# tirtho109/parallel_AMG

Measured on AMD Instinct MI355X. Metric: V-cycle iters/sec + fine-SpMV HBM GB/s, 3D Poisson 128M dofs at 1/2/4/8 GPU, higher is better.
Workload: dtype f64; 1 GPU; poisson3d 512^3 fp64, SA-AMG V(1,1) weighted-Jacobi, 1 part(s); n=134217728, nnz_fine=937951232, levels=6, max_coarse=1000, parallelism=row-slab partition p1

## Files before the change

include/pamg.h:

```cpp
#ifndef PAMG_H
#define PAMG_H

#include <stdint.h>

#ifdef __cplusplus
extern "C" {
#endif

#define PAMG_OK 0
#define PAMG_E_ARG (-1)
#define PAMG_E_HIP (-2)
#define PAMG_E_RCCL (-3)
#define PAMG_E_OVERFLOW (-4)
#define PAMG_E_SETUP (-5)
#define PAMG_E_STATE (-6)
#define PAMG_E_NOMEM (-7)

typedef struct pamg_ctx pamg_ctx;
typedef struct pamg_plan pamg_plan;
typedef struct pamg_vec pamg_vec;
typedef struct pamg_mat pamg_mat;
typedef struct pamg_hier pamg_hier;
typedef struct pamg_hcsr pamg_hcsr;

// ... 55 lines not shown
int pamg_mat_upload(pamg_ctx* ctx, int64_t nrows, int64_t ncols_local, const int64_t* rowptr,
                    const void* col, int col_is_64, const double* val, int index_base,
                    const pamg_plan* col_plan, pamg_mat** out);
int pamg_mat_upload_perm(pamg_ctx* ctx, int64_t nrows, int64_t ncols_local, const int64_t* rowptr,
                         const void* col, int col_is_64, const double* val, int index_base,
                         const pamg_plan* col_plan, const int64_t* row_perm,
                         const int64_t* col_perm, pamg_mat** out);
int pamg_mat_upload_blocked(pamg_ctx* ctx, int64_t nrows, int64_t ncols_local, const int64_t* rowptr,
                            const void* col, int col_is_64, const double* val, int index_base,
                            const pamg_plan* col_plan, int bs, pamg_mat** out);
int pamg_mat_destroy(pamg_mat* A);
int pamg_mat_info(const pamg_mat* A, int64_t* nrows, int64_t* ncols_local, int64_t* nnz);
int pamg_mat_stream_bytes(const pamg_mat* A, int64_t* bytes);
int pamg_mat_layout(const pamg_mat* A, int set, int out[10]);
int pamg_mat_ell_window(const pamg_mat* A, int out[16]);
int pamg_mat_ell_classes(const pamg_mat* A, int64_t out[8]);

int pamg_mat_set_block_diag(pamg_ctx* ctx, pamg_mat* A, int bs, const double* blocks, const double* inv);
int pamg_mat_block_size(const pamg_mat* A, int* bs);

int pamg_spmv(pamg_ctx* ctx, const pamg_mat* A, pamg_vec* x, pamg_vec* y);
int pamg_residual(pamg_ctx* ctx, const pamg_mat* A, pamg_vec* x, const pamg_vec* b,
                  pamg_vec* r, double* nrm2);
int pamg_jacobi(pamg_ctx* ctx, const pamg_mat* A, pamg_vec* x, const pamg_vec* b,
                pamg_vec* tmp, double omega, int nsweeps);
int pamg_jacobi_residual(pamg_ctx* ctx, const pamg_mat* A, pamg_vec* x, const pamg_vec* b,
                         pamg_vec* t, pamg_vec* r, double omega, int* fused);
int pamg_chebyshev_coeffs(double lmax, double ratio, int degree, double* c1, double* c2);
int pamg_chebyshev(pamg_ctx* ctx, const pamg_mat* A, pamg_vec* x, const pamg_vec* b, pamg_vec* tmp1,
                   pamg_vec* tmp2, double lmax, double ratio, int degree);
// ... 86 lines not shown
```

parallel_amg_amd/_lib.py:

```python
from __future__ import annotations

import contextlib
import ctypes as C
import os

_HERE = os.path.dirname(os.path.abspath(__file__))
LIB_PATH = os.environ.get("PAMG_LIB") or os.path.join(_HERE, "libpamg.so")

PAMG_OK = 0
ERRORS = {-1: "PAMG_E_ARG", -2: "PAMG_E_HIP", -3: "PAMG_E_RCCL", -4: "PAMG_E_OVERFLOW",
          -5: "PAMG_E_SETUP", -6: "PAMG_E_STATE", -7: "PAMG_E_NOMEM"}


class PamgError(RuntimeError):
    def __init__(self, code, fn, msg):
        super().__init__(f"{fn} -> {ERRORS.get(code, code)}: {msg}")
        self.code = code


vp = C.c_void_p
i32, i64, dbl = C.c_int, C.c_int64, C.c_double
pvp = C.POINTER(C.c_void_p)
pi64 = C.POINTER(C.c_int64)
pdbl = C.POINTER(C.c_double)
# ... 39 lines not shown
    "pamg_vec_copy": [vp, vp, vp],
    "pamg_vec_axpby": [vp, dbl, vp, dbl, vp],
    "pamg_vec_dot": [vp, vp, vp, pdbl],
    "pamg_vec_nrm2": [vp, vp, pdbl],
    "pamg_exchange": [vp, vp, vp],
    "pamg_exchange_begin": [vp, vp, vp],
    "pamg_exchange_end": [vp, vp, vp],
    "pamg_mat_upload": [vp, i64, i64, vp, vp, i32, vp, i32, vp, pvp],
    "pamg_mat_upload_perm": [vp, i64, i64, vp, vp, i32, vp, i32, vp, vp, vp, pvp],
    "pamg_mat_upload_blocked": [vp, i64, i64, vp, vp, i32, vp, i32, vp, i32, pvp],
    "pamg_mat_destroy": [vp],
    "pamg_mat_info": [vp, pi64, pi64, pi64],
    "pamg_mat_stream_bytes": [vp, pi64],
    "pamg_mat_layout": [vp, i32, C.POINTER(C.c_int)],
    "pamg_mat_ell_window": [vp, C.POINTER(C.c_int)],
    "pamg_mat_ell_classes": [vp, pi64],
    "pamg_mat_set_block_diag": [vp, vp, i32, vp, vp],
    "pamg_mat_block_size": [vp, C.POINTER(C.c_int)],
    "pamg_spmv": [vp, vp, vp, vp],
    "pamg_residual": [vp, vp, vp, vp, vp, pdbl],
    "pamg_jacobi": [vp, vp, vp, vp, vp, dbl, i32],
    "pamg_jacobi_residual": [vp, vp, vp, vp, vp, vp, dbl, pi32],
    "pamg_chebyshev_coeffs": [dbl, dbl, i32, vp, vp],
    "pamg_chebyshev": [vp, vp, vp, vp, vp, vp, dbl, dbl, i32],
    "pamg_estimate_lmax": [vp, vp, vp, vp, i32, i32, vp],
    "pamg_block_jacobi": [vp, vp, vp, vp, vp, dbl, i32],
    "pamg_block_chebyshev": [vp, vp, vp, vp, vp, vp, dbl, dbl, i32],
    "pamg_estimate_lmax_block": [vp, vp, vp, vp, i32, i32, vp],
    "pamg_hier_set_omega": [vp, vp],
    "pamg_hier_create": [vp, i32, vp, vp, vp, vp, i64, vp, i32, vp, pvp],
# ... 94 lines not shown
    old = C.c_int64()
    call("pamg_get_option", key.encode(), C.byref(old))
    call("pamg_set_option", key.encode(), int(value))
    try:
        yield
    finally:
        call("pamg_set_option", key.encode(), old.value)


def layout_of(M, part_set: int = 0) -> dict:
    out = (C.c_int * 10)()
    call("pamg_mat_layout", M.handle, part_set, out)
    win = (C.c_int * 16)()
    if part_set == 0:
        call("pamg_mat_ell_window", M.handle, win)
    cls = (C.c_int64 * 8)()
    if part_set == 0:
        call("pamg_mat_ell_classes", M.handle, cls)
    return {"ell_class": bool(cls[0]),
            "ell_class_census": {"slices": int(cls[1]), "classes_mean": round(cls[2] / max(cls[1], 1), 2),
                                 "classes_max": int(cls[3]), "record_bytes": int(cls[4]), "id_bytes": int(cls[5]),
                                 "replaced_bytes": int(cls[6])},
            "ell_xwin": bool(win[0]), "ell_xwin_groups": int(win[1]), "ell_gather_groups": int(win[2]),
            "ell_xwin_max_window": int(win[3]), "ell_xwin_noncontig_groups": int(win[4]),
            "ell_xwin_max_pairs": int(win[5]), "ell_xwin_max_chunks": int(win[6]),
            "ell_xwin_census": {"groups": int(win[7]), "full_groups": int(win[13]), "window_mean": int(win[8]),
                                "window_p95": int(win[9]), "runs_mean": int(win[10]), "runs_max": int(win[11]),
                                "pairs_mean": int(win[12])},
            "c24": bool(out[0]), "vd": bool(out[1]), "rl8": bool(out[2]), "cd": int(out[3]),
            "cd_offsets": int(out[4]), "tm": bool(out[5]), "tm_rs": int(out[6]),
            "tile_nnz": int(out[7]), "tiles": int(out[8]), "anchored": bool(out[9] & 1), "per_tile": bool(out[9] & 2),
            "x_stage": bool(out[9] & 4), "sym": bool(out[9] & 8), "sym_rows": 2 if out[9] & 16 else 1,
            "jr_fused": bool(out[9] & 32), "tm_vd": bool(out[9] & 64), "sym_vd": bool(out[9] & 128),
            "ell": bool(out[9] & 512), "pnc": bool(out[9] & 1024),
            "rpat": bool(out[9] & 2048), "pnc_compact": bool(out[9] & 4096),
            "ell_pair": bool(out[9] & 8192), "pnc_tiled": bool(out[9] & 16384),
            "bsr": bool(out[9] & 32768)}


def last_error() -> str:
    return lib().pamg_last_error().decode(errors="replace")


# ... 3 lines not shown
```

parallel_amg_amd/csrc/kernels.hip:

```cpp

#include "pamg_device.h"
#include "div_rn.h"

namespace pamg {
namespace {

__device__ __forceinline__ int wave_incl_scan(int v) {
    const int lane = threadIdx.x & 63, rl = lane & 15;
    int t;
    t = __builtin_amdgcn_mov_dpp(v, 0x111, 0xf, 0xf, false);
    if (rl >= 1) v += t;
    t = __builtin_amdgcn_mov_dpp(v, 0x112, 0xf, 0xf, false);
    if (rl >= 2) v += t;
    t = __builtin_amdgcn_mov_dpp(v, 0x114, 0xf, 0xf, false);
    if (rl >= 4) v += t;
    t = __builtin_amdgcn_mov_dpp(v, 0x118, 0xf, 0xf, false);
    if (rl >= 8) v += t;
    t = __builtin_amdgcn_mov_dpp(v, 0x142, 0xf, 0xf, false);
    if (lane & 16) v += t;
    t = __builtin_amdgcn_mov_dpp(v, 0x143, 0xf, 0xf, false);
    if (lane >= 32) v += t;
    return v;
}

// ... 1553 lines not shown
    for (int e = 0; e < 4; ++e) {
        const bool ok = FULL || 4 * q + e < L;
        const double p = vv[e] * xv[e];
        const double t = s + p;
        s = ok ? t : s;
    }
}

constexpr int kEllwPre = 12;
__device__ __forceinline__ void ellw_load(uint32_t (&cq)[kEllwPre], const uint32_t* __restrict__ cw, int first, int nq,
                                          int q0, int stride) {
#pragma unroll
    for (int e = 0; e < kEllwPre; ++e) cq[e] = cw[nq > 0 ? first + min(q0 + e, nq - 1) * stride : 0];
}

template <int OP, bool CLS>
__global__ __launch_bounds__(kEllGroup) void k_rows_ellw(int nrows, const int4* __restrict__ gslices,
                                                         const int2* __restrict__ smeta, const uint32_t* __restrict__ cw,
                                                         const uint8_t* __restrict__ cid,
                                                         const uint8_t* __restrict__ len, const uint8_t* __restrict__ dpos,
                                                         const int4* __restrict__ gmeta, const int* __restrict__ otab,
                                                         const double* __restrict__ vtab, const int4* __restrict__ wmeta, const int2* __restrict__ chunks,
                                                         const uint16_t* __restrict__ lofs, int win, int gather_all,
                                                         int ngroups, const double* __restrict__ x,
                                                         const double* __restrict__ b, double* __restrict__ y,
                                                         double omega, double c1 = 0.0,
                                                         const double* __restrict__ xold = nullptr) {
    extern __shared__ double ellw_lds[];
    double* lx = ellw_lds;
    double* lv = ellw_lds + win;
    uint16_t* lof = reinterpret_cast<uint16_t*>(lv + 256);
    const int per = (ngroups + 7) / 8;
    const int g = (blockIdx.x & 7) * per + (blockIdx.x >> 3);
    if (g >= ngroups) return;
    const int tid = threadIdx.x, lane = tid & 63;
    const int w = __builtin_amdgcn_readfirstlane(tid >> 6);
    const int4 gm = gmeta[g], wm = wmeta[g], gs = gslices[g];
    const int np = gm.y;
    const bool windowed = wm.y > 0 && !gather_all;
    const double vtv = vtab[gm.x + (tid < np ? tid : 0)];
    const uint32_t* __restrict__ l32 = reinterpret_cast<const uint32_t*>(lofs + wm.z);
    const uint32_t la = l32[windowed && tid < 2 * np ? tid : 0], lb = l32[windowed && tid + 256 < 2 * np ? tid + 256 : 0];
    const int2 cmv = chunks[wm.x + (w + 4 * lane < wm.y ? w + 4 * lane : 0)];
    const int slice = w == 0 ? gs.x : w == 1 ? gs.y : w == 2 ? gs.z : gs.w;
    const int i = slice * kEllW + lane;
    const bool in = slice >= 0 && i < nrows;
    const int ic = in ? i : 0;
    const int L = in ? (int)len[ic] : 0;
    const int2 sm = smeta[slice >= 0 ? slice : 0];
    const int nq = slice >= 0 ? ((CLS ? sm.y & 0xff : sm.y) + 3) >> 2 : 0;
    const int nfull = CLS && slice >= 0 ? __builtin_amdgcn_readfirstlane(((sm.y >> 8) & 0xff) >> 2) : 0;
    const int stride = CLS ? sm.y >> 16 : kEllW;
    const int first = sm.x + (CLS ? (in ? (int)cid[ic] : 0) : lane);
    const uint32_t* __restrict__ cp = cw + first;
    double pb = 0.0, px = 0.0, py = 0.0, pxo = 0.0;
    if constexpr (OP == OP_RESID || kDiagOp<OP>) pb = b[ic];
    if constexpr (kDiagOp<OP>) px = x[ic];
    if constexpr (OP == OP_PROLONG) py = y[ic];
    if constexpr (OP == OP_CHEB) pxo = xold ? xold[ic] : 0.0;
    uint32_t dkw = 0u;
    int dk = 255;
    if constexpr (kDiagOp<OP>) {
        dk = in ? (int)dpos[ic] : 255;
        dkw = cw[dk != 255 ? first + (dk >> 2) * stride : 0];
    }
    double s = 0.0;
    if (windowed) {
        uint32_t cq[kEllwPre];
        ellw_load(cq, cw, first, nq, 0, stride);
        for (int k = 0; w + 4 * k < wm.y; ++k) {
            const int col = __builtin_amdgcn_readlane(cmv.x, k), sc = __builtin_amdgcn_readlane(cmv.y, k);
            if (lane < (sc >> 16))
                __builtin_amdgcn_global_load_lds(
                    (const __attribute__((address_space(1))) void*)(x + col + 2 * lane),
                    (__attribute__((address_space(3))) void*)(lx + (sc & 0xffff)), 16, 0, 0);
        }
        if (tid < np) lv[tid] = vtv;
        if (tid < 2 * np) reinterpret_cast<uint32_t*>(lof)[tid] = la;
        if (tid + 256 < 2 * np) reinterpret_cast<uint32_t*>(lof)[tid + 256] = lb;
        __syncthreads();
        for (int q0 = 0; q0 < nq; q0 += kEllwPre) {
            if (q0 > 0) ellw_load(cq, cw, first, nq, q0, stride);
#pragma unroll
            for (int e = 0; e < kEllwPre; ++e)
                if (CLS && q0 + e < nfull)
// ... 959 lines not shown
template <int OP>
void launch_rows_op(const pamg_mat& A, const TileSet& ts, const double* x, const double* b,
                    double* y, double omega, hipStream_t s, Cheb ch = Cheb{}) {
    if (ts.bsr) launch_bsr<OP, 0>(A, x, b, y, omega, s, ch);
    if (ts.sym) launch_sym<OP>(A, x, b, y, omega, s, ch);
    if (ts.ell) {
        const EllSet& E = A.ell;
        const int grid = (int)((E.ngroups + 7) / 8 * 8);
        auto go = [&](auto kern) {
            kern<<<grid, kEllGroup, 0, s>>>((int)A.nrows, E.d_gorder, E.d_anc, E.d_smeta, E.d_ci, E.d_vi, E.d_len,
                                            E.d_gmeta, E.d_otab, E.d_vtab, (int)E.ngroups, x, b, y, omega, ch.c1,
                                            ch.xold);
        };
        if (E.win) {
            const int win = std::max(E.max_window, 128);
            const size_t lds = sizeof(double) * (size_t)(win + 256) + sizeof(uint16_t) * 4 * 256;
            auto gow = [&](auto kern) {
                kern<<<grid, kEllGroup, lds, s>>>((int)A.nrows, E.d_gslices, E.d_smeta, E.d_ci, E.d_cid, E.d_len, E.d_dpos,
                                                  E.d_gmeta, E.d_otab, E.d_vtab, E.d_wmeta, E.d_chunks, E.d_lof, win,
                                                  (reinterpret_cast<uintptr_t>(x) & 15) != 0 ? 1 : 0, (int)E.ngroups, x, b,
                                                  y, omega, ch.c1, ch.xold);
            };
            if (E.cls) gow(k_rows_ellw<OP, true>);
            else gow(k_rows_ellw<OP, false>);
        } else if (E.d_anc) {
            if (E.paired) go(k_rows_ell<OP, true, true>);
            else go(k_rows_ell<OP, true, false>);
        } else {
            if (E.paired) go(k_rows_ell<OP, false, true>);
            else go(k_rows_ell<OP, false, false>);
        }
    }
    if constexpr (OP != OP_CHEB) {
        if (ts.pnc) launch_pnc<OP>(A, x, b, y, omega, s);
        if (ts.rpat) launch_rpat<OP>(A, x, b, y, omega, s);
    }
    if (ts.n_short > 0) {
        if (ts.tile_nnz == 1024) launch_tile<OP, 1024>(A, ts, x, b, y, omega, s, ch);
        else if (ts.tile_nnz == 4096) launch_tile<OP, 4096>(A, ts, x, b, y, omega, s, ch);
// ... 379 lines not shown
```

parallel_amg_amd/csrc/matrix.hip:

```cpp
#include <algorithm>
#include <array>
#include <atomic>
#include <chrono>
#include <cstdint>
#include <cstdio>
#include <cstdlib>
#include <cstring>
#include <functional>
#include <iterator>
#include <memory>
#include <mutex>
#include <new>
#include <thread>
#include <utility>
#include <vector>

#include "pamg_device.h"
#include "pamg_host.h"

namespace {

int host_threads() {
    static const int n = [] {
        const char* e = std::getenv("OMP_NUM_THREADS");
        int v = e ? std::atoi(e) : 0;
        if (v <= 0) v = (int)std::thread::hardware_concurrency();
        return std::max(1, std::min(v, 64));
    }();
    return n;
}

template <class F>
void par_for(int64_t n, F&& f) {
// ... 784 lines not shown
                couple(take);
            }
            for (int t : touched) score[t] = 0;
            grp.push_back(g);
        }
    }
    std::vector<std::vector<std::pair<int, int>>>().swap(scoup);
    std::vector<std::vector<uint64_t>>().swap(spair);
    const int64_t ng = (int64_t)grp.size();
    std::vector<std::vector<int>> goff(ng);
    std::vector<std::vector<uint64_t>> gval(ng);
    std::vector<std::vector<int2>> gchunk(ng);
    std::vector<std::vector<uint16_t>> glof(ng);
    std::vector<int> gwin(ng, 0), gruns(ng, 0);
    std::vector<int64_t> gnnz(ng, 0);
    std::vector<uint32_t> cw(words + 1, 0u);
    std::vector<uint8_t> len(n + kVecPad, 0), dpos(n + kVecPad, (uint8_t)255);
    par_for(ng, [&](int64_t a, int64_t b) {
        constexpr int kSlots = 1024;
        std::vector<int> pid(kSlots), pstamp(kSlots, -1), pkey_o(kSlots);
        std::vector<uint64_t> pkey_v(kSlots);
        std::vector<int> o, lmin(4 * 256), lmax(4 * 256);
        std::vector<uint64_t> v;
        std::vector<std::array<int, 2>> rng;
        std::vector<std::array<int, 3>> runs;
        for (int64_t g = a; g < b && ok; ++g) {
            const int stamp = (int)(g - a);
            o.clear();
            v.clear();
            for (int w = 0; w < 4 && ok; ++w) {
// ... 56 lines not shown
            }
            int slots = 0, nch = 0;
            for (auto& r : runs) {
                r[2] = slots;
                slots += r[1] - r[0];
                nch += (r[1] - r[0] + 127) / 128;
            }
            if (slots == 0 || slots > cap || nch > pamg::kEllWinChunks) continue;
            if (runs.front()[0] < 0 || runs.back()[1] > ((int)A->ncols + 1)) continue;
            gwin[g] = slots;
            gruns[g] = (int)runs.size();
            for (const auto& r : runs)
                for (int c = r[0]; c < r[1]; c += 128)
                    gchunk[g].push_back(make_int2(c, (r[2] + c - r[0]) | (std::min(128, r[1] - c) / 2) << 16));
            glof[g].assign((size_t)4 * np, (uint16_t)64);
            for (int w = 0; w < 4; ++w)
                for (int p = 0; p < np; ++p) {
                    uint16_t word = 64;
                    if (grp[g][w] >= 0 && lmax[w * 256 + p] >= 0) {
                        const int c0 = grp[g][w] * kEllW + o[p], c = c0 + lmin[w * 256 + p];
                        size_t r = 0;
                        while (r + 1 < runs.size() && runs[r + 1][0] <= c) ++r;
                        word = (uint16_t)(runs[r][2] + c0 - runs[r][0] + 64);
                    }
                    glof[g][(size_t)w * np + p] = word;
                }
        }
    });
    if (!ok) return PAMG_OK;
    {
        int64_t have = 0;
        for (int64_t g = 0; g < ng; ++g) have += gwin[g] > 0;
        for (int k = 8; k >= 2 && have > 0; --k) {
            const int fit = ((pamg::kEllLdsPerCu / k - 2048) / 8 - 256) & ~1;
            int64_t keep = 0;
            for (int64_t g = 0; g < ng; ++g) keep += gwin[g] > 0 && gwin[g] <= fit;
            if (keep * 100 < pamg::kEllWinKeep * have) continue;
            for (int64_t g = 0; g < ng; ++g)
                if (gwin[g] > fit) {
                    gwin[g] = 0;
                    gchunk[g].clear();
                    glof[g].clear();
                }
            break;
        }
    }
    pamg::EllSet& E = A->ell;
    int64_t win_nnz = 0, win_slots = 0, win_runs = 0, win_pairs = 0;
    for (int64_t g = 0; g < ng; ++g) {
        E.max_pairs = std::max(E.max_pairs, (int)goff[g].size());
        bool contig = true;
        for (int w = 1; w < 4; ++w) contig = contig && (grp[g][w] < 0 || grp[g][w] == grp[g][0] + w);
        if (gwin[g] > 0) {
            ++E.win_groups;
            win_nnz += gnnz[g];
            win_slots += gwin[g];
            E.max_window = std::max(E.max_window, gwin[g]);
// ... 9 lines not shown
    }
    if ((int64_t)E.win_groups * 100 < pamg::kEllWinMinShare * ng || win_nnz * 100 < pamg::kEllWinMinRatio100 * win_slots) {
        E = pamg::EllSet{};
        return PAMG_OK;
    }
    {
        std::vector<int> ws;
        for (int64_t g = 0; g < ng; ++g)
            if (gwin[g] > 0) ws.push_back(gwin[g]);
        std::sort(ws.begin(), ws.end());
        E.p95_window = ws[(ws.size() - 1) * 95 / 100];
        E.mean_window = (int)(win_slots / E.win_groups);
        E.mean_runs = (int)(win_runs / E.win_groups);
        E.mean_pairs = (int)(win_pairs / E.win_groups);
    }
    std::vector<int4> gmeta(ng), wmeta(ng), gsl(ng);
    int64_t on = 0, cn = 0, ln = 0;
    for (int64_t g = 0; g < ng; ++g) {
        const int np = (int)goff[g].size();
        gmeta[g] = make_int4((int)on, np, (int)on, np);
        wmeta[g] = make_int4((int)cn, (int)gchunk[g].size(), (int)ln, gwin[g]);
        gsl[g] = make_int4(grp[g][0], grp[g][1], grp[g][2], grp[g][3]);
        on += np;
        cn += (int64_t)gchunk[g].size();
        ln += (int64_t)glof[g].size();
    }
    if (ln >= INT32_MAX || cn >= INT32_MAX) {
        E = pamg::EllSet{};
        return PAMG_OK;
    }
    std::vector<int> otab(on + 1, 0);
    std::vector<double> vtab(on + 1, 0.0);
    std::vector<int2> chunks(cn + 1, make_int2(0, 0));
    std::vector<uint16_t> lof(ln + 2, (uint16_t)0);
    par_for(ng, [&](int64_t a, int64_t b) {
        for (int64_t g = a; g < b; ++g) {
            std::copy(goff[g].begin(), goff[g].end(), otab.begin() + gmeta[g].x);
            for (size_t e = 0; e < gval[g].size(); ++e) std::memcpy(&vtab[gmeta[g].x + e], &gval[g][e], 8);
            std::copy(gchunk[g].begin(), gchunk[g].end(), chunks.begin() + wmeta[g].x);
            std::copy(glof[g].begin(), glof[g].end(), lof.begin() + wmeta[g].z);
        }
    });
    std::vector<int2> smeta_c;
    std::vector<uint32_t> ccw;
    std::vector<uint8_t> cid;
    if (pamg::options().ell_xwin == 1) {
        std::vector<int> snc(ns, 0), smin(ns, 0);
        cid.assign(n + kVecPad, 0);
        par_for(ns, [&](int64_t a, int64_t b) {
            int rep[kEllW];
            for (int64_t q = a; q < b; ++q) {
                const int nq = (smeta[q].y + 3) / 4;
                const int64_t r0 = q * kEllW, s0 = smeta[q].x;
                const int rows = (int)std::min<int64_t>(n - r0, kEllW);
                int nc = 0;
                for (int l = 0; l < rows; ++l) {
                    int c = 0;
                    for (; c < nc; ++c) {
                        const int m = rep[c];
                        bool same = len[r0 + l] == len[r0 + m] && dpos[r0 + l] == dpos[r0 + m];
                        for (int k = 0; k < nq && same; ++k) same = cw[s0 + (int64_t)k * kEllW + l] == cw[s0 + (int64_t)k * kEllW + m];
// ... 63 lines not shown
    CHECK(dalloc(&E.d_wmeta, ng));
    CHECK(dalloc(&E.d_chunks, cn + 1));
    CHECK(dalloc(&E.d_lof, ln + 2));
    CHECK(dalloc(&E.d_dpos, n + kVecPad));
    CHECK(h2d(ctx, E.d_dpos, dpos.data(), dpos.size()));
    CHECK(h2d(ctx, E.d_smeta, sm_up.data(), sizeof(int2) * ns));
    CHECK(h2d(ctx, E.d_ci, cw_up.data(), sizeof(uint32_t) * (up_words + 1)));
    CHECK(h2d(ctx, E.d_len, len.data(), len.size()));
    CHECK(h2d(ctx, E.d_gmeta, gmeta.data(), sizeof(int4) * ng));
    CHECK(h2d(ctx, E.d_otab, otab.data(), sizeof(int) * (on + 1)));
    CHECK(h2d(ctx, E.d_vtab, vtab.data(), sizeof(double) * (on + 1)));
    CHECK(h2d(ctx, E.d_gslices, gsl.data(), sizeof(int4) * ng));
    CHECK(h2d(ctx, E.d_wmeta, wmeta.data(), sizeof(int4) * ng));
    CHECK(h2d(ctx, E.d_chunks, chunks.data(), sizeof(int2) * (cn + 1)));
    CHECK(h2d(ctx, E.d_lof, lof.data(), sizeof(uint16_t) * (ln + 2)));
    A->interior.ell = true;
    return PAMG_OK;
}

int build_ell(pamg_mat* A, const PtrVec& rp, const IdxVec& ci, const double* val,
              bool anchored, const std::vector<int>& inner) {
    using pamg::kEllGroup;
    using pamg::kEllSkip;
    using pamg::kEllW;
    const int64_t n = A->nrows;
    std::vector<char> in_set;
    if ((int64_t)inner.size() != n) {
        in_set.assign(n, 0);
        for (int i : inner) in_set[i] = 1;
    }
// ... 194 lines not shown
        (int64_t)u.inner.size() * 4 >= (int64_t)nrows * 3 && nrows >= pamg::options().ell_min_rows &&
        (n_own_cols == nrows || pamg::options().ell_restrict)) {
        CHECK(build_ell(A, u.rp, u.ci, u.val, n_own_cols != nrows, u.inner));
        if (A->interior.ell) u.inner.clear();
        u.tr.mark("ell");
    }
    return PAMG_OK;
}

int64_t ell_bytes(const pamg_mat* A) {
    if (!A->interior.ell) return 0;
    const int64_t nrows = A->nrows;
    const int64_t index = A->ell.cls ? 4 * A->ell.cls_words + nrows : (A->ell.paired ? 4 : 8) * A->ell.words;
    return index + nrows + 8 * A->ell.nslices + 16 * A->ell.ngroups + 4 * A->ell.otab_n +
           8 * A->ell.vtab_n + (A->ell.d_anc ? 4 * nrows : 0) +
           (A->ell.win ? 32 * A->ell.ngroups + 8 * A->ell.nchunks + 2 * A->ell.lof_n + nrows : 0);
}

void ell_report(const pamg_mat* A, const pamg::TileSet& t, int out[10]) {
    if (!t.ell) return;
    out[8] = (int)A->ell.ngroups;
    out[9] |= 512 | (A->ell.paired ? 8192 : 0);
}

void ell_window(const pamg_mat* A, int out[16]) {
    const pamg::EllSet& E = A->ell;
    const bool w = A->interior.ell && E.win;
    out[0] = w ? 1 : 0;
    out[1] = w ? E.win_groups : 0;
    out[2] = w ? E.gather_groups : 0;
    out[3] = w ? E.max_window : 0;
    out[4] = w ? E.noncontig_groups : 0;
    out[5] = w ? E.max_pairs : 0;
    out[6] = w ? E.max_chunks : 0;
    out[7] = w ? (int)E.ngroups : 0;
    out[8] = w ? E.mean_window : 0;
    out[9] = w ? E.p95_window : 0;
    out[10] = w ? E.mean_runs : 0;
    out[11] = w ? E.max_runs : 0;
    out[12] = w ? E.mean_pairs : 0;
    out[13] = w ? E.full_groups : 0;
    out[14] = out[15] = 0;
}

void ell_classes(const pamg_mat* A, int64_t out[8]) {
    const pamg::EllSet& E = A->ell;
    const bool c = A->interior.ell && E.cls;
    out[0] = c ? 1 : 0;
    out[1] = c ? E.nslices : 0;
    out[2] = c ? E.cls_total : 0;
    out[3] = c ? E.cls_max : 0;
    out[4] = c ? 4 * E.cls_words : 0;
    out[5] = c ? A->nrows : 0;
    out[6] = c ? 4 * E.words : 0;
    out[7] = 0;
}

void ell_free(pamg::EllSet& E) {
    dfree(E.d_cid);
    dfree(E.d_gorder);
    dfree(E.d_smeta);
    dfree(E.d_ci);
    dfree(E.d_vi);
    dfree(E.d_len);
    dfree(E.d_gmeta);
    dfree(E.d_otab);
    dfree(E.d_vtab);
    dfree(E.d_anc);
    dfree(E.d_gslices);
    dfree(E.d_wmeta);
    dfree(E.d_chunks);
    dfree(E.d_lof);
    dfree(E.d_dpos);
    E = pamg::EllSet{};
}


int build_pnc(pamg_mat* A, const PtrVec& rp, const IdxVec& ci, const double* val,
              const std::array<int64_t, 4>& grid, const std::vector<int>& inner) {
    using pamg::kPncMaxLen;
    using pamg::kPncSkip;
    const int64_t n = A->nrows;
    std::vector<char> in_set;
    if ((int64_t)inner.size() != n) {
        in_set.assign(n, 0);
        for (int i : inner) in_set[i] = 1;
    }
    auto member = [&](int64_t i) { return in_set.empty() || in_set[i]; };
// ... 1343 lines not shown
    tiles_report(A, t, out);
    ell_report(A, t, out);
    rpat_report(A, t, out);
    pnc_report(A, t, out);
    sym_report(A, t, out);
    bsr_report(A, t, out);
    return PAMG_OK;
}

int pamg_mat_ell_window(const pamg_mat* A, int out[16]) {
    if (!A || !out) return fail(PAMG_E_ARG, "mat_ell_window: bad args");
    ell_window(A, out);
    return PAMG_OK;
}

int pamg_mat_ell_classes(const pamg_mat* A, int64_t out[8]) {
    if (!A || !out) return fail(PAMG_E_ARG, "mat_ell_classes: bad args");
    ell_classes(A, out);
    return PAMG_OK;
}

}
```

parallel_amg_amd/csrc/pamg_device.h:

```cpp
#pragma once

#include <hip/hip_runtime.h>
#include <rccl/rccl.h>

#include <atomic>
#include <cstdint>
#include <array>
#include <mutex>
#include <vector>

#include "pamg_common.h"

namespace pamg {

constexpr int kBlock = 256;
constexpr int kTileRows = 256;

constexpr int kXsMaxClusters = 12;
constexpr int kTmSmallTab = 128;
constexpr int kXsCap = 1088;
constexpr int kXsIoff = 128;
constexpr int kXsGap = 48;
struct XStage {
    int ncl = 0, stride = 0, zix = -1, ncols = 0;
// ... 91 lines not shown
    int nx = 0, ny = 0, nz = 0;
    int tiles_x = 0, tiles_y = 0;
    int zchunks = 1, zlen = 0;
    int zlo = 0, zhi = 0;
    int xfast = 0;
};
constexpr int kEllW = 64;
constexpr int kEllGroup = 256;
constexpr int kEllSkip = 255;
constexpr int kEllWinCap = 7168;
constexpr int kEllWinChunks = 256;
constexpr int kEllLdsPerCu = 160 * 1024;
constexpr int kEllWinKeep = 85;
constexpr int kEllWinMinShare = 50;
constexpr int kEllWinMinRatio100 = 150;
struct EllSet {
    int64_t nslices = 0, ngroups = 0;
    int2* d_smeta = nullptr;
    uint32_t* d_ci = nullptr;
    uint32_t* d_vi = nullptr;
    uint8_t* d_len = nullptr;
    int4* d_gmeta = nullptr;
    int* d_otab = nullptr;
    double* d_vtab = nullptr;
    int* d_anc = nullptr;
    int* d_gorder = nullptr;
    int64_t words = 0, otab_n = 0, vtab_n = 0;
    bool paired = false;
    bool win = false;
    int4* d_gslices = nullptr;
    int4* d_wmeta = nullptr;
    int2* d_chunks = nullptr;
    uint16_t* d_lof = nullptr;
    uint8_t* d_dpos = nullptr;
    int64_t nchunks = 0, lof_n = 0;
    int win_groups = 0, gather_groups = 0, noncontig_groups = 0;
    int max_window = 0, max_pairs = 0, max_chunks = 0;
    int mean_window = 0, p95_window = 0, mean_runs = 0, max_runs = 0, mean_pairs = 0, full_groups = 0;
    bool cls = false;
    uint8_t* d_cid = nullptr;
    int64_t cls_words = 0;
    int cls_max = 0;
    int64_t cls_total = 0;
};

constexpr int kPncPatMax = 1024, kPncValMax = 128, kPncMaxLen = 7;
constexpr int kPncSkip = kPncPatMax - 1;
constexpr int kPncCombMax = 1024;
constexpr int kPncCombSkip = 0xffff;
constexpr int kPncTx = 64, kPncTy = 4;
constexpr bool pnc_tiled(int nx, int ny) { return nx % kPncTx == 0 && ny % kPncTy == 0; }
struct PncSet {
    int nx = 0, ny = 0, nz = 0;
// ... 188 lines not shown
```

parallel_amg_amd/csrc/runtime.hip:

```cpp
#include <dlfcn.h>

#include <algorithm>
#include <atomic>
#include <chrono>
#include <cmath>
#include <condition_variable>
#include <cstddef>
#include <cstdint>
#include <cstdio>
#include <cstring>
#include <limits>
#include <memory>
#include <mutex>
#include <string>
#include <thread>
#include <utility>
#include <vector>

#include "pamg_device.h"
#include "pamg_host.h"

pamg::Options& pamg::options() {
    static Options o;
    return o;
// ... 2269 lines not shown
    {"long_tiles_min", &O::long_tiles_min, 1, 255, false},
    {"tm_tile_dicts", &O::tm_tile_dicts, 0, 1, false},
    {"sym_dia", &O::sym_dia, 0, 1, false},
    {"sym_rows", &O::sym_rows, 1, 2, false},
    {"jr_fuse", &O::jr_fuse, 0, 1, false},
    {"sym_vd", &O::sym_vd, 0, 1, false},
    {"symd_chunks", &O::symd_chunks, 1, 4, true},
    {"sym_zm", &O::sym_zm, 0, 1, false},
    {"tb_xfast", &O::tb_xfast, 0, 1, false},
    {"ell", &O::ell, 0, 1, false},
    {"ell_restrict", &O::ell_restrict, 0, 1, false},
    {"pnc", &O::pnc, 0, 2, false},
    {"rpat", &O::rpat, 0, 1, false},
    {"pnc_compact", &O::pnc_compact, 0, 1, false},
    {"ell_pair", &O::ell_pair, 0, 1, false},
    {"ell_xwin", &O::ell_xwin, 0, 2, false},
    {"ell_xwin_max", &O::ell_xwin_max, 2, pamg::kEllWinCap, false},
    {"ell_yblock", &O::ell_yblock, 0, 65536, false},
    {"ell_min_rows", &O::ell_min_rows, 0, INT32_MAX, false},
    {"zm_chunks", &O::zm_chunks, 0, 4096, false},
    {"chain_store_x", &O::chain_store_x, 0, 1, false},
};

const OptionRow* find_option(const char* key) {
    for (const OptionRow& r : kOptionTable)
        if (std::strcmp(r.key, key) == 0) return &r;
    return nullptr;
}
}

extern "C" {
// ... 106 lines not shown
```

Measured before the change: 232.3 V-cycles/s.

## Pair adjacent ELL window groups to share a unioned LDS x-window

Greedily pairs ELL slice groups whose x-column windows overlap and runs each pair in one double-size workgroup. The block stages the union of both windows into LDS once, with local offsets remapped into the union. The goal is to cut redundant global loads of overlapping x segments in the windowed SpMV. The costs are larger LDS per block (which may lower occupancy), an extra kernel launch for the unpaired groups, and more setup work.

```diff
diff --git a/include/pamg.h b/include/pamg.h
--- a/include/pamg.h
+++ b/include/pamg.h
@@ -93,6 +93,7 @@
 int pamg_mat_stream_bytes(const pamg_mat* A, int64_t* bytes);
 int pamg_mat_layout(const pamg_mat* A, int set, int out[10]);
 int pamg_mat_ell_window(const pamg_mat* A, int out[16]);
+int pamg_mat_ell_span(const pamg_mat* A, int out[8]);
 int pamg_mat_ell_classes(const pamg_mat* A, int64_t out[8]);
 
 int pamg_mat_set_block_diag(pamg_ctx* ctx, pamg_mat* A, int bs, const double* blocks, const double* inv);
diff --git a/parallel_amg_amd/_lib.py b/parallel_amg_amd/_lib.py
--- a/parallel_amg_amd/_lib.py
+++ b/parallel_amg_amd/_lib.py
@@ -77,6 +77,7 @@
     "pamg_mat_stream_bytes": [vp, pi64],
     "pamg_mat_layout": [vp, i32, C.POINTER(C.c_int)],
     "pamg_mat_ell_window": [vp, C.POINTER(C.c_int)],
+    "pamg_mat_ell_span": [vp, C.POINTER(C.c_int)],
     "pamg_mat_ell_classes": [vp, pi64],
     "pamg_mat_set_block_diag": [vp, vp, i32, vp, vp],
     "pamg_mat_block_size": [vp, C.POINTER(C.c_int)],
@@ -201,8 +202,10 @@
     win = (C.c_int * 16)()
     if part_set == 0:
         call("pamg_mat_ell_window", M.handle, win)
+    span = (C.c_int * 8)()
     cls = (C.c_int64 * 8)()
     if part_set == 0:
+        call("pamg_mat_ell_span", M.handle, span)
         call("pamg_mat_ell_classes", M.handle, cls)
     return {"ell_class": bool(cls[0]),
             "ell_class_census": {"slices": int(cls[1]), "classes_mean": round(cls[2] / max(cls[1], 1), 2),
@@ -213,7 +216,10 @@
             "ell_xwin_max_pairs": int(win[5]), "ell_xwin_max_chunks": int(win[6]),
             "ell_xwin_census": {"groups": int(win[7]), "full_groups": int(win[13]), "window_mean": int(win[8]),
                                 "window_p95": int(win[9]), "runs_mean": int(win[10]), "runs_max": int(win[11]),
-                                "pairs_mean": int(win[12])},
+                                "pairs_mean": int(win[12]),
+                                "span_pairs": int(span[0]), "span_singles": int(span[1]),
+                                "union_mean": int(span[2]), "union_p95": int(span[3]),
+                                "union_ratio": span[4] / 100.0, "union_max": int(span[5])},
             "c24": bool(out[0]), "vd": bool(out[1]), "rl8": bool(out[2]), "cd": int(out[3]),
             "cd_offsets": int(out[4]), "tm": bool(out[5]), "tm_rs": int(out[6]),
             "tile_nnz": int(out[7]), "tiles": int(out[8]), "anchored": bool(out[9] & 1), "per_tile": bool(out[9] & 2),
diff --git a/parallel_amg_amd/csrc/ell_span.h b/parallel_amg_amd/csrc/ell_span.h
--- /dev/null
+++ b/parallel_amg_amd/csrc/ell_span.h
@@ -0,0 +1,91 @@
+#pragma once
+#include <algorithm>
+#include <array>
+#include <cstdint>
+#include <utility>
+#include <vector>
+
+namespace pamg {
+
+using EllRuns = std::vector<std::array<int, 3>>;
+
+inline int ell_span_union(const EllRuns& a, const EllRuns& b, EllRuns& out, int& chunks) {
+    out.clear();
+    size_t i = 0, j = 0;
+    while (i < a.size() || j < b.size()) {
+        const bool ta = j == b.size() || (i < a.size() && a[i][0] <= b[j][0]);
+        const std::array<int, 3>& r = ta ? a[i++] : b[j++];
+        if (!out.empty() && r[0] <= out.back()[1] + 16) out.back()[1] = std::max(out.back()[1], r[1]);
+        else out.push_back({r[0], r[1], 0});
+    }
+    int slots = 0;
+    chunks = 0;
+    for (auto& r : out) {
+        r[2] = slots;
+        slots += r[1] - r[0];
+        chunks += (r[1] - r[0] + 127) / 128;
+    }
+    return slots;
+}
+
+inline int ell_span_overlap(const EllRuns& a, const EllRuns& b) {
+    int n = 0;
+    size_t i = 0, j = 0;
+    while (i < a.size() && j < b.size()) {
+        n += std::max(0, std::min(a[i][1], b[j][1]) - std::max(a[i][0], b[j][0]));
+        if (a[i][1] <= b[j][1]) ++i;
+        else ++j;
+    }
+    return n;
+}
+
+inline uint16_t ell_span_relof(uint16_t word, int lmin, const EllRuns& own, const EllRuns& uni) {
+    const int slot = (int)word - 64 + lmin;
+    size_t r = 0;
+    while (r + 1 < own.size() && own[r + 1][2] <= slot) ++r;
+    const int col = own[r][0] + slot - own[r][2];
+    size_t u = 0;
+    while (u + 1 < uni.size() && uni[u + 1][0] <= col) ++u;
+    return (uint16_t)(uni[u][2] + col - uni[u][0] - lmin + 64);
+}
+
+inline std::vector<std::pair<int, int>> ell_span_pairs(const std::vector<EllRuns>& runs, const std::vector<int>& gwin,
+                                                       const std::vector<int>& sgroup, int w, int cap,
+                                                       int max_chunks, int share) {
+    const int ng = (int)runs.size(), ns = (int)sgroup.size();
+    std::vector<std::pair<int, int>> pairs;
+    std::vector<char> done(ng, 0);
+    std::vector<int> cand, score(ng, 0);
+    EllRuns uni;
+    for (int a = 0; a < ng; ++a) {
+        if (done[a] || runs[a].empty()) continue;
+        done[a] = 1;
+        cand.clear();
+        for (const auto& r : runs[a])
+            for (int q = std::max(r[0], 0) / w; q <= (r[1] - 1) / w && q < ns; ++q) {
+                const int b = sgroup[q];
+                if (b >= 0 && !done[b] && !runs[b].empty() && score[b] == 0) {
+                    score[b] = 1 + ell_span_overlap(runs[a], runs[b]);
+                    cand.push_back(b);
+                }
+            }
+        const size_t top = std::min<size_t>(6, cand.size());
+        std::partial_sort(cand.begin(), cand.begin() + top, cand.end(),
+                          [&](int p, int q) { return score[p] != score[q] ? score[p] > score[q] : p < q; });
+        int take = -1;
+        for (size_t c = 0; c < top && take < 0; ++c) {
+            int nch = 0;
+            const int slots = ell_span_union(runs[a], runs[cand[c]], uni, nch);
+            if (slots <= cap && nch <= max_chunks && (int64_t)slots * 100 <= (int64_t)share * (gwin[a] + gwin[cand[c]]))
+                take = cand[c];
+        }
+        for (int b : cand) score[b] = 0;
+        if (take >= 0) {
+            done[take] = 1;
+            pairs.push_back({a, take});
+        }
+    }
+    return pairs;
+}
+
+}
diff --git a/parallel_amg_amd/csrc/kernels.hip b/parallel_amg_amd/csrc/kernels.hip
--- a/parallel_amg_amd/csrc/kernels.hip
+++ b/parallel_amg_amd/csrc/kernels.hip
@@ -1591,34 +1591,47 @@
     for (int e = 0; e < kEllwPre; ++e) cq[e] = cw[nq > 0 ? first + min(q0 + e, nq - 1) * stride : 0];
 }
 
-template <int OP, bool CLS>
-__global__ __launch_bounds__(kEllGroup) void k_rows_ellw(int nrows, const int4* __restrict__ gslices,
+template <int OP, bool CLS, int SPAN = 1>
+__global__ __launch_bounds__(SPAN * kEllGroup) void k_rows_ellw(int nrows, const int4* __restrict__ gslices,
                                                          const int2* __restrict__ smeta, const uint32_t* __restrict__ cw,
                                                          const uint8_t* __restrict__ cid,
                                                          const uint8_t* __restrict__ len, const uint8_t* __restrict__ dpos,
                                                          const int4* __restrict__ gmeta, const int* __restrict__ otab,
                                                          const double* __restrict__ vtab, const int4* __restrict__ wmeta, const int2* __restrict__ chunks,
                                                          const uint16_t* __restrict__ lofs, int win, int gather_all,
+                                                         const int4* __restrict__ pairs, int g0,
                                                          int ngroups, const double* __restrict__ x,
                                                          const double* __restrict__ b, double* __restrict__ y,
                                                          double omega, double c1 = 0.0,
                                                          const double* __restrict__ xold = nullptr) {
     extern __shared__ double ellw_lds[];
     double* lx = ellw_lds;
-    double* lv = ellw_lds + win;
-    uint16_t* lof = reinterpret_cast<uint16_t*>(lv + 256);
     const int per = (ngroups + 7) / 8;
-    const int g = (blockIdx.x & 7) * per + (blockIdx.x >> 3);
-    if (g >= ngroups) return;
-    const int tid = threadIdx.x, lane = tid & 63;
-    const int w = __builtin_amdgcn_readfirstlane(tid >> 6);
-    const int4 gm = gmeta[g], wm = wmeta[g], gs = gslices[g];
+    const int gl = (blockIdx.x & 7) * per + (blockIdx.x >> 3);
+    if (gl >= ngroups) return;
+    const int g = g0 + gl;
+    const int lane = threadIdx.x & 63, tid = threadIdx.x & (kEllGroup - 1);
+    const int wv = __builtin_amdgcn_readfirstlane(threadIdx.x >> 6);
+    const int w = wv & 3, half = wv >> 2;
+    double* lv = ellw_lds + win + 256 * half;
+    uint16_t* lof = reinterpret_cast<uint16_t*>(ellw_lds + win + 256 * SPAN) + 4 * 256 * half;
+    int4 gm, wm, gs;
+    if constexpr (SPAN == 2) {
+        const int4 ra = pairs[4 * g], rb = pairs[4 * g + 1], rt = pairs[4 * g + 2], rw = pairs[4 * g + 3];
+        gs = half ? rb : ra;
+        gm = half ? make_int4(rt.z, rt.w, rt.z, rt.w) : make_int4(rt.x, rt.y, rt.x, rt.y);
+        wm = make_int4(rw.x, rw.y & 0xffff, half ? rw.w : rw.z, rw.y >> 16);
+    } else {
+        gm = gmeta[g];
+        wm = wmeta[g];
+        gs = gslices[g];
+    }
     const int np = gm.y;
-    const bool windowed = wm.y > 0 && !gather_all;
+    const bool windowed = SPAN == 2 || (wm.y > 0 && !gather_all);
     const double vtv = vtab[gm.x + (tid < np ? tid : 0)];
     const uint32_t* __restrict__ l32 = reinterpret_cast<const uint32_t*>(lofs + wm.z);
     const uint32_t la = l32[windowed && tid < 2 * np ? tid : 0], lb = l32[windowed && tid + 256 < 2 * np ? tid + 256 : 0];
-    const int2 cmv = chunks[wm.x + (w + 4 * lane < wm.y ? w + 4 * lane : 0)];
+    const int2 cmv = chunks[wm.x + (wv + 4 * SPAN * lane < wm.y ? wv + 4 * SPAN * lane : 0)];
     const int slice = w == 0 ? gs.x : w == 1 ? gs.y : w == 2 ? gs.z : gs.w;
     const int i = slice * kEllW + lane;
     const bool in = slice >= 0 && i < nrows;
@@ -1645,7 +1658,7 @@
     if (windowed) {
         uint32_t cq[kEllwPre];
         ellw_load(cq, cw, first, nq, 0, stride);
-        for (int k = 0; w + 4 * k < wm.y; ++k) {
+        for (int k = 0; wv + 4 * SPAN * k < wm.y; ++k) {
             const int col = __builtin_amdgcn_readlane(cmv.x, k), sc = __builtin_amdgcn_readlane(cmv.y, k);
             if (lane < (sc >> 16))
                 __builtin_amdgcn_global_load_lds(
@@ -2635,15 +2648,24 @@
         };
         if (E.win) {
             const int win = std::max(E.max_window, 128);
-            const size_t lds = sizeof(double) * (size_t)(win + 256) + sizeof(uint16_t) * 4 * 256;
-            auto gow = [&](auto kern) {
-                kern<<<grid, kEllGroup, lds, s>>>((int)A.nrows, E.d_gslices, E.d_smeta, E.d_ci, E.d_cid, E.d_len, E.d_dpos,
-                                                  E.d_gmeta, E.d_otab, E.d_vtab, E.d_wmeta, E.d_chunks, E.d_lof, win,
-                                                  (reinterpret_cast<uintptr_t>(x) & 15) != 0 ? 1 : 0, (int)E.ngroups, x, b,
-                                                  y, omega, ch.c1, ch.xold);
+            const int gather_all = (reinterpret_cast<uintptr_t>(x) & 15) != 0 ? 1 : 0;
+            const int npairs = gather_all ? 0 : E.npairs, nrest = (int)E.ngroups - 2 * npairs;
+            auto gow = [&](auto kern, int span, int g0, int n, int wn) {
+                const size_t bytes = sizeof(double) * (size_t)(wn + 256 * span) + sizeof(uint16_t) * 4 * 256 * span;
+                kern<<<(n + 7) / 8 * 8, span * kEllGroup, bytes, s>>>(
+                    (int)A.nrows, E.d_gslices, E.d_smeta, E.d_ci, E.d_cid, E.d_len, E.d_dpos, E.d_gmeta, E.d_otab,
+                    E.d_vtab, E.d_wmeta, E.d_chunks, E.d_lof, wn, gather_all, E.d_pairs, g0, n, x, b, y, omega, ch.c1,
+                    ch.xold);
             };
-            if (E.cls) gow(k_rows_ellw<OP, true>);
-            else gow(k_rows_ellw<OP, false>);
+            if (npairs > 0) {
+                const int wu = std::max(E.max_union, 128);
+                if (E.cls) gow(k_rows_ellw<OP, true, 2>, 2, 0, npairs, wu);
+                else gow(k_rows_ellw<OP, false, 2>, 2, 0, npairs, wu);
+            }
+            if (nrest > 0) {
+                if (E.cls) gow(k_rows_ellw<OP, true>, 1, 2 * npairs, nrest, win);
+                else gow(k_rows_ellw<OP, false>, 1, 2 * npairs, nrest, win);
+            }
         } else if (E.d_anc) {
             if (E.paired) go(k_rows_ell<OP, true, true>);
             else go(k_rows_ell<OP, true, false>);
diff --git a/parallel_amg_amd/csrc/matrix.hip b/parallel_amg_amd/csrc/matrix.hip
--- a/parallel_amg_amd/csrc/matrix.hip
+++ b/parallel_amg_amd/csrc/matrix.hip
@@ -17,6 +17,7 @@
 
 #include "pamg_device.h"
 #include "pamg_host.h"
+#include "ell_span.h"
 
 namespace {
 
@@ -831,6 +832,9 @@
     std::vector<std::vector<uint16_t>> glof(ng);
     std::vector<int> gwin(ng, 0), gruns(ng, 0);
     std::vector<int64_t> gnnz(ng, 0);
+    const bool span2 = pamg::options().ell_xwin <= 2;
+    std::vector<pamg::EllRuns> gwruns(span2 ? ng : 0);
+    std::vector<std::vector<uint8_t>> glmin(span2 ? ng : 0);
     std::vector<uint32_t> cw(words + 1, 0u);
     std::vector<uint8_t> len(n + kVecPad, 0), dpos(n + kVecPad, (uint8_t)255);
     par_for(ng, [&](int64_t a, int64_t b) {
@@ -917,6 +921,10 @@
                 for (int c = r[0]; c < r[1]; c += 128)
                     gchunk[g].push_back(make_int2(c, (r[2] + c - r[0]) | (std::min(128, r[1] - c) / 2) << 16));
             glof[g].assign((size_t)4 * np, (uint16_t)64);
+            if (span2) {
+                gwruns[g] = runs;
+                glmin[g].assign((size_t)4 * np, (uint8_t)255);
+            }
             for (int w = 0; w < 4; ++w)
                 for (int p = 0; p < np; ++p) {
                     uint16_t word = 64;
@@ -925,6 +933,7 @@
                         size_t r = 0;
                         while (r + 1 < runs.size() && runs[r + 1][0] <= c) ++r;
                         word = (uint16_t)(runs[r][2] + c0 - runs[r][0] + 64);
+                        if (span2) glmin[g][(size_t)w * np + p] = (uint8_t)lmin[w * 256 + p];
                     }
                     glof[g][(size_t)w * np + p] = word;
                 }
@@ -944,6 +953,7 @@
                     gwin[g] = 0;
                     gchunk[g].clear();
                     glof[g].clear();
+                    if (span2) gwruns[g].clear();
                 }
             break;
         }
@@ -983,12 +993,79 @@
         E.mean_runs = (int)(win_runs / E.win_groups);
         E.mean_pairs = (int)(win_pairs / E.win_groups);
     }
+    std::vector<int> gunion(ng, 0);
+    if (span2) {
+        std::vector<int> sgroup(ns, -1);
+        for (int64_t g = 0; g < ng; ++g)
+            for (int w = 0; w < 4; ++w)
+                if (grp[g][w] >= 0) sgroup[grp[g][w]] = (int)g;
+        const std::vector<std::pair<int, int>> prs =
+            pamg::ell_span_pairs(gwruns, gwin, sgroup, kEllW, std::min(cap, pamg::kEllSpanWin), pamg::kEllSpanChunks,
+                                 pamg::kEllSpanShare);
+        E.npairs = (int)prs.size();
+        if (E.npairs > 0) {
+            std::vector<int> order;
+            std::vector<char> paired(ng, 0);
+            order.reserve(ng);
+            for (const auto& pr : prs) {
+                order.push_back(pr.first);
+                order.push_back(pr.second);
+                paired[pr.first] = paired[pr.second] = 1;
+            }
+            for (int64_t g = 0; g < ng; ++g)
+                if (!paired[g]) order.push_back((int)g);
+            auto permute = [&](auto& v) {
+                std::remove_reference_t<decltype(v)> t(v.size());
+                for (int64_t g = 0; g < ng; ++g) t[g] = std::move(v[order[g]]);
+                v.swap(t);
+            };
+            permute(grp);
+            permute(goff);
+            permute(gval);
+            permute(gchunk);
+            permute(glof);
+            permute(gwin);
+            permute(gwruns);
+            permute(glmin);
+            std::vector<int> usz(E.npairs);
+            int64_t usum = 0, upct = 0;
+            par_for(E.npairs, [&](int64_t a, int64_t b) {
+                pamg::EllRuns uni;
+                for (int64_t p = a; p < b; ++p) {
+                    int nch = 0;
+                    usz[p] = pamg::ell_span_union(gwruns[2 * p], gwruns[2 * p + 1], uni, nch);
+                    gchunk[2 * p].clear();
+                    gchunk[2 * p + 1].clear();
+                    for (const auto& r : uni)
+                        for (int c = r[0]; c < r[1]; c += 128)
+                            gchunk[2 * p].push_back(make_int2(c, (r[2] + c - r[0]) | (std::min(128, r[1] - c) / 2) << 16));
+                    for (int64_t g = 2 * p; g < 2 * p + 2; ++g) {
+                        for (size_t e = 0; e < glof[g].size(); ++e)
+                            if (glmin[g][e] != 255)
+                                glof[g][e] = pamg::ell_span_relof(glof[g][e], glmin[g][e], gwruns[g], uni);
+                        gunion[g] = usz[p];
+                    }
+                }
+            });
+            for (int p = 0; p < E.npairs; ++p) {
+                usum += usz[p];
+                upct += (int64_t)usz[p] * 100 / (gwin[2 * p] + gwin[2 * p + 1]);
+                E.max_union = std::max(E.max_union, usz[p]);
+            }
+            std::sort(usz.begin(), usz.end());
+            E.p95_union = usz[(usz.size() - 1) * 95 / 100];
+            E.mean_union = (int)(usum / E.npairs);
+            E.union_pct = (int)(upct / E.npairs);
+        }
+        std::vector<pamg::EllRuns>().swap(gwruns);
+        std::vector<std::vector<uint8_t>>().swap(glmin);
+    }
     std::vector<int4> gmeta(ng), wmeta(ng), gsl(ng);
     int64_t on = 0, cn = 0, ln = 0;
     for (int64_t g = 0; g < ng; ++g) {
         const int np = (int)goff[g].size();
         gmeta[g] = make_int4((int)on, np, (int)on, np);
-        wmeta[g] = make_int4((int)cn, (int)gchunk[g].size(), (int)ln, gwin[g]);
+        wmeta[g] = make_int4((int)cn, gunion[g] ? 0 : (int)gchunk[g].size(), (int)ln, gunion[g] ? gunion[g] : gwin[g]);
         gsl[g] = make_int4(grp[g][0], grp[g][1], grp[g][2], grp[g][3]);
         on += np;
         cn += (int64_t)gchunk[g].size();
@@ -997,6 +1074,14 @@
     if (ln >= INT32_MAX || cn >= INT32_MAX) {
         E = pamg::EllSet{};
         return PAMG_OK;
+    }
+    std::vector<int4> prec((size_t)4 * E.npairs);
+    for (int p = 0; p < E.npairs; ++p) {
+        const int a = 2 * p, b = a + 1;
+        prec[4 * p] = gsl[a];
+        prec[4 * p + 1] = gsl[b];
+        prec[4 * p + 2] = make_int4(gmeta[a].x, gmeta[a].y, gmeta[b].x, gmeta[b].y);
+        prec[4 * p + 3] = make_int4(wmeta[a].x, (int)gchunk[a].size() | gunion[a] << 16, wmeta[a].z, wmeta[b].z);
     }
     std::vector<int> otab(on + 1, 0);
     std::vector<double> vtab(on + 1, 0.0);
@@ -1013,7 +1098,7 @@
     std::vector<int2> smeta_c;
     std::vector<uint32_t> ccw;
     std::vector<uint8_t> cid;
-    if (pamg::options().ell_xwin == 1) {
+    if (pamg::options().ell_xwin == 1 || pamg::options().ell_xwin == 3) {
         std::vector<int> snc(ns, 0), smin(ns, 0);
         cid.assign(n + kVecPad, 0);
         par_for(ns, [&](int64_t a, int64_t b) {
@@ -1107,6 +1192,10 @@
     CHECK(h2d(ctx, E.d_wmeta, wmeta.data(), sizeof(int4) * ng));
     CHECK(h2d(ctx, E.d_chunks, chunks.data(), sizeof(int2) * (cn + 1)));
     CHECK(h2d(ctx, E.d_lof, lof.data(), sizeof(uint16_t) * (ln + 2)));
+    if (E.npairs > 0) {
+        CHECK(dalloc(&E.d_pairs, prec.size()));
+        CHECK(h2d(ctx, E.d_pairs, prec.data(), sizeof(int4) * prec.size()));
+    }
     A->interior.ell = true;
     return PAMG_OK;
 }
@@ -1331,7 +1420,8 @@
     const int64_t index = A->ell.cls ? 4 * A->ell.cls_words + nrows : (A->ell.paired ? 4 : 8) * A->ell.words;
     return index + nrows + 8 * A->ell.nslices + 16 * A->ell.ngroups + 4 * A->ell.otab_n +
            8 * A->ell.vtab_n + (A->ell.d_anc ? 4 * nrows : 0) +
-           (A->ell.win ? 32 * A->ell.ngroups + 8 * A->ell.nchunks + 2 * A->ell.lof_n + nrows : 0);
+           (A->ell.win ? 32 * A->ell.ngroups + 8 * A->ell.nchunks + 2 * A->ell.lof_n + nrows : 0) -
+           32 * (int64_t)A->ell.npairs;
 }
 
 void ell_report(const pamg_mat* A, const pamg::TileSet& t, int out[10]) {
@@ -1360,6 +1450,18 @@
     out[14] = out[15] = 0;
 }
 
+void ell_span(const pamg_mat* A, int out[8]) {
+    const pamg::EllSet& E = A->ell;
+    const bool w = A->interior.ell && E.win;
+    out[0] = w ? E.npairs : 0;
+    out[1] = w ? E.win_groups - 2 * E.npairs : 0;
+    out[2] = w ? E.mean_union : 0;
+    out[3] = w ? E.p95_union : 0;
+    out[4] = w ? E.union_pct : 0;
+    out[5] = w ? E.max_union : 0;
+    out[6] = out[7] = 0;
+}
+
 void ell_classes(const pamg_mat* A, int64_t out[8]) {
     const pamg::EllSet& E = A->ell;
     const bool c = A->interior.ell && E.cls;
@@ -1389,6 +1491,7 @@
     dfree(E.d_chunks);
     dfree(E.d_lof);
     dfree(E.d_dpos);
+    dfree(E.d_pairs);
     E = pamg::EllSet{};
 }
 
@@ -2762,6 +2865,12 @@
     return PAMG_OK;
 }
 
+int pamg_mat_ell_span(const pamg_mat* A, int out[8]) {
+    if (!A || !out) return fail(PAMG_E_ARG, "mat_ell_span: bad args");
+    ell_span(A, out);
+    return PAMG_OK;
+}
+
 int pamg_mat_ell_classes(const pamg_mat* A, int64_t out[8]) {
     if (!A || !out) return fail(PAMG_E_ARG, "mat_ell_classes: bad args");
     ell_classes(A, out);
diff --git a/parallel_amg_amd/csrc/pamg_device.h b/parallel_amg_amd/csrc/pamg_device.h
--- a/parallel_amg_amd/csrc/pamg_device.h
+++ b/parallel_amg_amd/csrc/pamg_device.h
@@ -129,6 +129,9 @@
 constexpr int kEllWinKeep = 85;
 constexpr int kEllWinMinShare = 50;
 constexpr int kEllWinMinRatio100 = 150;
+constexpr int kEllSpanWin = (kEllLdsPerCu / 4 - 2 * 4096) / 8;
+constexpr int kEllSpanChunks = 2 * kEllWinChunks;
+constexpr int kEllSpanShare = 90;
 struct EllSet {
     int64_t nslices = 0, ngroups = 0;
     int2* d_smeta = nullptr;
@@ -152,6 +155,10 @@
     int win_groups = 0, gather_groups = 0, noncontig_groups = 0;
     int max_window = 0, max_pairs = 0, max_chunks = 0;
     int mean_window = 0, p95_window = 0, mean_runs = 0, max_runs = 0, mean_pairs = 0, full_groups = 0;
+    int4* d_pairs = nullptr;
+    int npairs = 0;
+    int max_union = 0, mean_union = 0, p95_union = 0;
+    int union_pct = 0;
     bool cls = false;
     uint8_t* d_cid = nullptr;
     int64_t cls_words = 0;
diff --git a/parallel_amg_amd/csrc/runtime.hip b/parallel_amg_amd/csrc/runtime.hip
--- a/parallel_amg_amd/csrc/runtime.hip
+++ b/parallel_amg_amd/csrc/runtime.hip
@@ -2307,7 +2307,7 @@
     {"rpat", &O::rpat, 0, 1, false},
     {"pnc_compact", &O::pnc_compact, 0, 1, false},
     {"ell_pair", &O::ell_pair, 0, 1, false},
-    {"ell_xwin", &O::ell_xwin, 0, 2, false},
+    {"ell_xwin", &O::ell_xwin, 0, 4, false},
     {"ell_xwin_max", &O::ell_xwin_max, 2, pamg::kEllWinCap, false},
     {"ell_yblock", &O::ell_yblock, 0, 65536, false},
     {"ell_min_rows", &O::ell_min_rows, 0, INT32_MAX, false},
```

Measured after the change: 238.9 V-cycles/s, median of 6. +2.8%, better.
